# speedinghzl/DSRG

Hardware: AMD Instinct MI355X
Metric: images/sec DSRG train step (VGG16 321x321, 21-class) (higher is better)
Workload: dtype bf16 backbone (fp32 master weights) + f32/f64 supervision path

## Files before the change

### dsrg_amd/csrc/conv_igemm.hip

```cpp
#include "common.h"
#include <algorithm>
#include <cstdlib>
#include <cstring>
#include <functional>
#include <map>
#include <mutex>
#include <queue>
#include <vector>

namespace dsrg {
namespace {
typedef __attribute__((ext_vector_type(8))) __bf16 bf16x8;
typedef __attribute__((ext_vector_type(2))) __bf16 bf16x2;
typedef __attribute__((ext_vector_type(2))) float f32x2;
typedef __attribute__((ext_vector_type(16))) float f32x16;
typedef __attribute__((address_space(3))) void lds_void;

constexpr int kBM = 256, kBN = 256;
constexpr int kOutRow = 128 * 2 + 16;
constexpr int kOutWave = 64 * kOutRow;
constexpr uint32_t kOob = 0x80000000u;
constexpr int kRowTab = 8 * kOutWave;
constexpr int kRowTabBytes = kBM * 4;

__device__ __forceinline__ void wait_vm_lgkm_barrier() {
    asm volatile("s_waitcnt vmcnt(0) lgkmcnt(0)\n\ts_barrier" ::: "memory");
}

template <int BK, int NST> struct ICfg {
    static constexpr int ROW = BK * 2;
    static constexpr int CPR = ROW / 16;
    static constexpr int RPI = 1024 / ROW;
    static constexpr int IPW = 256 / RPI / 8;
    static constexpr int STAGE = (kBM + kBN) * ROW;
    static constexpr int KS = BK / 16;
    static constexpr int SPC = 64 / BK;
    static constexpr int AHEAD = NST - 1;
    static_assert(NST * STAGE <= kRowTab, "the row table sits behind the stages");
    static constexpr size_t LDS = (size_t)kRowTab + kRowTabBytes;
    __device__ static constexpr int swz(int r) { return BK == 64 ? (r >> 1) & 7 : (r >> 2) & 3; }
};

// ... 36 lines not shown
}
__device__ __forceinline__ uint32_t dropout_bytes(uint32_t e4, uint32_t seed_lo, uint32_t seed_hi) {
    return fmix32(fmix32(e4 ^ seed_lo) + seed_hi);
}

__device__ __forceinline__ uint32_t pack2(float lo, float hi) {
    f32x2 v = {lo, hi};
    bf16x2 b = __builtin_convertvector(v, bf16x2);
    return *reinterpret_cast<uint32_t *>(&b);
}

template <int N> __device__ __forceinline__ void wait_vm_barrier() {
    asm volatile("s_waitcnt vmcnt(%0)\n\ts_barrier" ::"n"(N) : "memory");
}

template <int BK, int NST, bool EARLY = false>
__device__ __forceinline__ void conv_igemm_body(const IgemmArgs &a, const int bid, const int nblk) {
    using C = ICfg<BK, NST>;
    extern __shared__ __attribute__((aligned(16))) unsigned char ig_lds[];
    const int tid = threadIdx.x, lane = tid & 63;
    const int wv = __builtin_amdgcn_readfirstlane(tid >> 6);
    const int l31 = lane & 31, kgrp = lane >> 5;
    const int wn = wv >> 2, wm = wv & 3;

    int grp, tm, tn;
    if (a.xcd_mix) {
        const int id = bid, xcd = id & 7, k = id >> 3;
        const int cm = (a.tiles_m - xcd + 7) >> 3, per_group = cm * a.tiles_n;
        if (cm <= 0 || k >= per_group * a.ngroups) return;
        grp = k / per_group;
        const int r = k - grp * per_group, tml = r / a.tiles_n;
        tn = r - tml * a.tiles_n;
        tm = xcd + 8 * tml;
    } else {
        const int total = nblk, id = bid;
        const int q = total >> 3, r = total & 7, xcd = id & 7, k = id >> 3;
        int t = (xcd < r ? xcd * (q + 1) : r * (q + 1) + (xcd - r) * q) + k;
// ... 100 lines not shown
        if (taps == 9) { dy = tap / 3 - 1; dx = tap - (tap / 3) * 3 - 1; }
        const int xc = a.cpp ? (int)((0x610u >> (2 * (cc / a.cpp))) & 3u) * a.cpp + cc % a.cpp : cc;
        const int toff = (dy * G.dil * W + dx * G.dil) * xrow + xc * 128 + h * C::ROW;
        unsigned char *P = ig_lds + stage * C::STAGE + wv * (32 * C::ROW);
        unsigned char *Wt = P + kBM * C::ROW;
#pragma unroll
        for (int i = 0; i < C::IPW; i++) {
            const uint32_t vo = ((pvalid[i] >> tap) & 1u) ? pbase[i] + (uint32_t)toff : kOob;
            __builtin_amdgcn_raw_ptr_buffer_load_lds(rx, (lds_void *)(P + i * (C::RPI * C::ROW)), 16, vo, 0, 0, 0);
        }
#pragma unroll
        for (int i = 0; i < C::IPW; i++)
            __builtin_amdgcn_raw_ptr_buffer_load_lds(rw, (lds_void *)(Wt + i * (C::RPI * C::ROW)), 16, wbase[i], s_real * C::ROW, 0, 0);
    };

    f32x16 acc[4][2];
#pragma unroll
    for (int i = 0; i < 4; i++)
#pragma unroll
        for (int j = 0; j < 2; j++)
#pragma unroll
            for (int r = 0; r < 16; r++) acc[i][j][r] = 0.0f;

    const int sw = C::swz(l31);
    const uint32_t rowoff = (uint32_t)l31 * C::ROW;
    uint32_t choff[C::KS];
#pragma unroll
    for (int ks = 0; ks < C::KS; ks++) choff[ks] = rowoff + (uint32_t)(((ks * 2 + kgrp) ^ sw) << 4);

    const bool active = n0 + wn * 128 < a.Cout;
    constexpr int LPS = 2 * C::IPW;
    if (EARLY) {
        static_assert(!EARLY || NST == 2, "the early-barrier schedule is written for two stages");
        bf16x8 af[2][4], bfr[2][2];
        const bool late = a.stagger && wv >= 4 && active;
        issue(0, 0);
        if (nsteps > 1) { issue(1, 1); wait_vm_barrier<LPS>(); } else { wait_vm_barrier<0>(); }
        if (active) {
            const unsigned char *P = ig_lds + wm * (64 * C::ROW), *Wt = ig_lds + kBM * C::ROW + wn * (128 * C::ROW);
#pragma unroll
            for (int i = 0; i < 4; i++) af[0][i] = *reinterpret_cast<const bf16x8 *>(Wt + i * (32 * C::ROW) + choff[0]);
#pragma unroll
            for (int j = 0; j < 2; j++) bfr[0][j] = *reinterpret_cast<const bf16x8 *>(P + j * (32 * C::ROW) + choff[0]);
        }
        for (int s = 0; s < nsteps; s++) {
            const int stage = s & 1;
            const bool next = s + 1 < nsteps, more = s + 2 < nsteps;
            if (!active) {
                if (next) { wait_vm_lgkm_barrier(); if (more) issue(stage, s + 2); }
                continue;
            }
            const unsigned char *P = ig_lds + stage * C::STAGE + wm * (64 * C::ROW);
            const unsigned char *Wt = ig_lds + stage * C::STAGE + kBM * C::ROW + wn * (128 * C::ROW);
            const unsigned char *Pn = ig_lds + (stage ^ 1) * C::STAGE + wm * (64 * C::ROW);
            const unsigned char *Wn = ig_lds + (stage ^ 1) * C::STAGE + kBM * C::ROW + wn * (128 * C::ROW);
#pragma unroll
            for (int ks = 0; ks < C::KS; ks++) {
                if (ks + 1 < C::KS) {
#pragma unroll
                    for (int i = 0; i < 4; i++) af[(ks + 1) & 1][i] = *reinterpret_cast<const bf16x8 *>(Wt + i * (32 * C::ROW) + choff[ks + 1 < C::KS ? ks + 1 : 0]);
#pragma unroll
                    for (int j = 0; j < 2; j++) bfr[(ks + 1) & 1][j] = *reinterpret_cast<const bf16x8 *>(P + j * (32 * C::ROW) + choff[ks + 1 < C::KS ? ks + 1 : 0]);
                } else if (next) {
                    wait_vm_lgkm_barrier();
                    if (more && !late) issue(stage, s + 2);
#pragma unroll
                    for (int i = 0; i < 4; i++) af[C::KS & 1][i] = *reinterpret_cast<const bf16x8 *>(Wn + i * (32 * C::ROW) + choff[0]);
#pragma unroll
                    for (int j = 0; j < 2; j++) bfr[C::KS & 1][j] = *reinterpret_cast<const bf16x8 *>(Pn + j * (32 * C::ROW) + choff[0]);
                }
                __builtin_amdgcn_sched_barrier(0);
#pragma unroll
                for (int i = 0; i < 4; i++)
#pragma unroll
                    for (int j = 0; j < 2; j++)
                        acc[i][j] = __builtin_amdgcn_mfma_f32_32x32x16_bf16(af[ks & 1][i], bfr[ks & 1][j], acc[i][j], 0, 0, 0);
                __builtin_amdgcn_sched_barrier(0);
                if (ks == C::KS - 1 && more && late) issue(stage, s + 2);
            }
        }
    } else {
#pragma unroll
    for (int p = 0; p < C::AHEAD; p++)
        if (p < nsteps) issue(p, p);
    int stage = 0;
    for (int s = 0; s < nsteps; s++) {
        if (C::AHEAD >= 3 && s + 2 < nsteps) wait_vm_barrier<2 * LPS>();
        else if (C::AHEAD >= 2 && s + 1 < nsteps) wait_vm_barrier<LPS>();
        else wait_vm_barrier<0>();
        const bool more = s + C::AHEAD < nsteps, late = a.stagger && wv >= 4 && active;
        const int nstage = stage == 0 ? NST - 1 : stage - 1;
        if (more && !late) issue(nstage, s + C::AHEAD);
        if (active) {
        const unsigned char *P = ig_lds + stage * C::STAGE + wm * (64 * C::ROW);
        const unsigned char *Wt = ig_lds + stage * C::STAGE + kBM * C::ROW + wn * (128 * C::ROW);
        bf16x8 af[2][4], bfr[2][2];
#pragma unroll
        for (int i = 0; i < 4; i++) af[0][i] = *reinterpret_cast<const bf16x8 *>(Wt + i * (32 * C::ROW) + choff[0]);
#pragma unroll
        for (int j = 0; j < 2; j++) bfr[0][j] = *reinterpret_cast<const bf16x8 *>(P + j * (32 * C::ROW) + choff[0]);
#pragma unroll
        for (int ks = 0; ks < C::KS; ks++) {
            if (ks + 1 < C::KS) {
#pragma unroll
                for (int i = 0; i < 4; i++) af[(ks + 1) & 1][i] = *reinterpret_cast<const bf16x8 *>(Wt + i * (32 * C::ROW) + choff[(ks + 1) % C::KS]);
#pragma unroll
                for (int j = 0; j < 2; j++) bfr[(ks + 1) & 1][j] = *reinterpret_cast<const bf16x8 *>(P + j * (32 * C::ROW) + choff[(ks + 1) % C::KS]);
            }
            __builtin_amdgcn_sched_barrier(0);
#pragma unroll
            for (int i = 0; i < 4; i++)
#pragma unroll
                for (int j = 0; j < 2; j++)
                    acc[i][j] = __builtin_amdgcn_mfma_f32_32x32x16_bf16(af[ks & 1][i], bfr[ks & 1][j], acc[i][j], 0, 0, 0);
            __builtin_amdgcn_sched_barrier(0);
            if (ks == 0 && more && late) issue(nstage, s + C::AHEAD);
        }
        }
        stage = stage + 1 == NST ? 0 : stage + 1;
    }
    }
    __syncthreads();
    if (!active) return;

    unsigned char *O = ig_lds + wv * kOutWave;
    const int nw = n0 + wn * 128;
    if (a.out_f32) {
        float *y32 = reinterpret_cast<float *>(G.y);
        const float floor32 = a.relu ? 0.0f : -__builtin_inff();
#pragma unroll
        for (int j = 0; j < 2; j++) {
            const int m = row_pixel(wm * 64 + j * 32 + l31);
#pragma unroll
            for (int i = 0; i < 4; i++)
#pragma unroll
                for (int q = 0; q < 4; q++) {
                    const int n = nw + i * 32 + q * 8 + kgrp * 4;
                    float4 b4 = make_float4(0.f, 0.f, 0.f, 0.f);
                    if (G.bias) b4 = *reinterpret_cast<const float4 *>(G.bias + n);
                    const float4 v = make_float4(fmaxf(acc[i][j][q * 4 + 0] + b4.x, floor32), fmaxf(acc[i][j][q * 4 + 1] + b4.y, floor32),
                                                 fmaxf(acc[i][j][q * 4 + 2] + b4.z, floor32), fmaxf(acc[i][j][q * 4 + 3] + b4.w, floor32));
                    if (m >= 0) *reinterpret_cast<float4 *>(y32 + (size_t)m * a.Cout + n) = v;
                }
        }
        return;
    }
    const rsrc_t rb = make_rsrc(G.bias, G.bias ? (size_t)a.Cout * 4 : 0);
    const float floor_ = (a.relu && !G.res) ? 0.0f : -__builtin_inff();
    const uint32_t seed_g = a.seed_lo + (uint32_t)grp * 0x9E3779B9u;
    float bias_r[4][4][4];
#pragma unroll
    for (int i = 0; i < 4; i++)
#pragma unroll
        for (int q = 0; q < 4; q++)
#pragma unroll
            for (int e = 0; e < 4; e++)
                bias_r[i][q][e] = ld_f32(rb, (uint32_t)(nw + i * 32 + q * 8 + kgrp * 4 + e) * 4u);
#pragma unroll
    for (int i = 0; i < 4; i++) {
#pragma unroll
        for (int q = 0; q < 4; q++) {
            const int nl = i * 32 + q * 8 + kgrp * 4;
            const float4 b4 = make_float4(bias_r[i][q][0], bias_r[i][q][1], bias_r[i][q][2], bias_r[i][q][3]);
#pragma unroll
            for (int j = 0; j < 2; j++) {
                float v0 = acc[i][j][q * 4 + 0] + b4.x, v1 = acc[i][j][q * 4 + 1] + b4.y;
                float v2 = acc[i][j][q * 4 + 2] + b4.z, v3 = acc[i][j][q * 4 + 3] + b4.w;
                v0 = fmaxf(v0, floor_) * a.out_scale; v1 = fmaxf(v1, floor_) * a.out_scale;
                v2 = fmaxf(v2, floor_) * a.out_scale; v3 = fmaxf(v3, floor_) * a.out_scale;
                if (a.drop_thresh) {
                    const uint32_t m = cls ? (uint32_t)rowpix[wm * 64 + j * 32 + l31] : (uint32_t)(m0 + wm * 64 + j * 32 + l31);
                    const uint32_t h = dropout_bytes((m * (uint32_t)a.Cout + (uint32_t)(nw + nl)) >> 2, seed_g, a.seed_hi);
                    v0 = (h & 0xffu) >= a.drop_thresh ? v0 * a.drop_scale : 0.0f;
                    v1 = ((h >> 8) & 0xffu) >= a.drop_thresh ? v1 * a.drop_scale : 0.0f;
                    v2 = ((h >> 16) & 0xffu) >= a.drop_thresh ? v2 * a.drop_scale : 0.0f;
                    v3 = (h >> 24) >= a.drop_thresh ? v3 * a.drop_scale : 0.0f;
                }
                *reinterpret_cast<uint2 *>(O + (j * 32 + l31) * kOutRow + nl * 2) = make_uint2(pack2(v0, v1), pack2(v2, v3));
            }
        }
    }
    const bool chv = nw + (lane & 15) * 8 < a.Cout;
    if (G.res) {
        const float floor2 = a.relu ? 0.0f : -__builtin_inff();
#pragma unroll
        for (int h = 0; h < 2; h++) {
            uint4 rs[8], mk8[8];
#pragma unroll
            for (int it = 0; it < 8; it++) {
                const int m = row_pixel(wm * 64 + (h * 8 + it) * 4 + (lane >> 4));
                const size_t at = (size_t)m * a.Cout + nw + (lane & 15) * 8;
                rs[it] = (m >= 0 && chv) ? *reinterpret_cast<const uint4 *>(G.res + at) : make_uint4(0, 0, 0, 0);
                mk8[it] = !G.mask ? make_uint4(0x3f803f80u, 0x3f803f80u, 0x3f803f80u, 0x3f803f80u)
                                  : ((m >= 0 && chv) ? *reinterpret_cast<const uint4 *>(G.mask + at) : make_uint4(0, 0, 0, 0));
// ... 71 lines not shown
        }
        __syncthreads();
        if (wm == 0) {
            const float *s0 = reinterpret_cast<const float *>(ig_lds + (wn * 4 + 0) * kOutWave);
            const float *s1 = reinterpret_cast<const float *>(ig_lds + (wn * 4 + 1) * kOutWave);
            const float *s2 = reinterpret_cast<const float *>(ig_lds + (wn * 4 + 2) * kOutWave);
            const float *s3 = reinterpret_cast<const float *>(ig_lds + (wn * 4 + 3) * kOutWave);
            float *dst = G.colsum + (size_t)tm * a.Cout + nw;
            dst[lane] = (s0[lane] + s1[lane]) + (s2[lane] + s3[lane]);
            if (nw + lane + 64 < a.Cout) dst[lane + 64] = (s0[lane + 64] + s1[lane + 64]) + (s2[lane + 64] + s3[lane + 64]);
        }
    }
}


__global__ __launch_bounds__(512, 2) void conv_igemm_kernel_64x2(IgemmArgs a) { conv_igemm_body<64, 2>(a, (int)blockIdx.x, (int)gridDim.x); }
__global__ __launch_bounds__(512, 2) void conv_igemm_kernel_64x2e(IgemmArgs a) { conv_igemm_body<64, 2, true>(a, (int)blockIdx.x, (int)gridDim.x); }
__global__ __launch_bounds__(512, 2) void conv_igemm_kernel_32x4(IgemmArgs a) { conv_igemm_body<32, 4>(a, (int)blockIdx.x, (int)gridDim.x); }

struct IgemmSkArgs {
    IgemmArgs base;
    float *ws;
    uint32_t *flags;
    int units, tiles_total;
};
constexpr int kSkParts = 4;
using f32x4v = decltype(__builtin_amdgcn_raw_buffer_load_b128(rsrc_t(), 0, 0, 0));

__global__ __launch_bounds__(512, 2) void conv_igemm_sk_kernel(IgemmSkArgs k) {
    using C = ICfg<64, 2>;
    const IgemmArgs &a = k.base;
    extern __shared__ __attribute__((aligned(16))) unsigned char ig_lds[];
    const int tid = threadIdx.x, lane = tid & 63;
    const int wv = __builtin_amdgcn_readfirstlane(tid >> 6);
    const int l31 = lane & 31, kgrp = lane >> 5;
    const int wn = wv >> 2, wm = wv & 3;
    int unit;
    {
        const int total = (int)gridDim.x, id = (int)blockIdx.x;
        const int q = total >> 3, r = total & 7, xcd = id & 7, kk = id >> 3;
        unit = (xcd < r ? xcd * (q + 1) : r * (q + 1) + (xcd - r) * q) + kk;
    }
    const int taps = a.taps, Cin = a.Cin, W = a.W, H = a.H;
    const int ktot = taps * Cin;
    const int nsteps = (Cin >> 6) * taps;
    const long long total_steps = (long long)k.tiles_total * nsteps;
    auto unit_start = [&](int u) { return (long long)u * total_steps / k.units; };
    const long long g1 = unit_start(unit + 1);
    const int sw = C::swz(l31);
    const uint32_t rowoff = (uint32_t)l31 * C::ROW;
    uint32_t choff[C::KS];
#pragma unroll
    for (int ks = 0; ks < C::KS; ks++) choff[ks] = rowoff + (uint32_t)(((ks * 2 + kgrp) ^ sw) << 4);
    const rsrc_t rws = make_rsrc(k.ws, (size_t)k.units * 32 * 512 * 16);
    const float floor_ = a.relu ? 0.0f : -__builtin_inff();

    for (long long g = unit_start(unit); g < g1;) {
        const int tile = (int)(g / nsteps);
        const int sb = (int)(g - (long long)tile * nsteps);
        const int se = (int)min((long long)nsteps, sb + (g1 - g));
        int t = tile;
        const int grp = t / a.tiles_per_group;
        t -= grp * a.tiles_per_group;
        const int tm = t / a.tiles_n, tn = t - tm * a.tiles_n;
        const int m0 = tm * kBM, n0 = tn * kBN;
        const IgemmGroup G = a.g[grp];
        const rsrc_t rx = make_rsrc(G.x, (size_t)a.M * Cin * 2);
        const rsrc_t rw = make_rsrc(G.w, (size_t)a.Cout * ktot * 2);
// ... 32 lines not shown
            const int toff = (dy * G.dil * W + dx * G.dil) * Cin * 2 + cc * 128;
            unsigned char *P = ig_lds + stage * C::STAGE + wv * (32 * C::ROW);
            unsigned char *Wt = P + kBM * C::ROW;
#pragma unroll
            for (int i = 0; i < C::IPW; i++) {
                const uint32_t bits = (i < 2 ? pvalid01 : pvalid23) >> (16 * (i & 1) + tap);
                const uint32_t off = ((pbase0 + (uint32_t)(i * C::RPI * Cin * 2)) ^ ((i & 1) ? 64u : 0u)) + (uint32_t)toff;
                __builtin_amdgcn_raw_ptr_buffer_load_lds(rx, (lds_void *)(P + i * (C::RPI * C::ROW)), 16, (bits & 1u) ? off : kOob, 0, 0, 0);
            }
#pragma unroll
            for (int i = 0; i < C::IPW; i++)
                __builtin_amdgcn_raw_ptr_buffer_load_lds(rw, (lds_void *)(Wt + i * (C::RPI * C::ROW)), 16, (i & 1) ? wbase0 ^ 64u : wbase0,
                                                         (uint32_t)s * C::ROW + (uint32_t)(i * C::RPI * ktot * 2), 0, 0);
        };

        f32x16 acc[4][2];
#pragma unroll
        for (int i = 0; i < 4; i++)
#pragma unroll
            for (int j = 0; j < 2; j++)
#pragma unroll
                for (int r = 0; r < 16; r++) acc[i][j][r] = 0.0f;

        issue(0, sb);
        for (int s = sb; s < se; s++) {
            const int stage = (s - sb) & 1;
            wait_vm_barrier<0>();
            const bool more = s + 1 < se, late = wv >= 4 && active;
            if (more && !late) issue(stage ^ 1, s + 1);
            if (active) {
                const unsigned char *P = ig_lds + stage * C::STAGE + wm * (64 * C::ROW);
                const unsigned char *Wt = ig_lds + stage * C::STAGE + kBM * C::ROW + wn * (128 * C::ROW);
                bf16x8 af[2][4], bfr[2][2];
#pragma unroll
                for (int i = 0; i < 4; i++) af[0][i] = *reinterpret_cast<const bf16x8 *>(Wt + i * (32 * C::ROW) + choff[0]);
#pragma unroll
                for (int j = 0; j < 2; j++) bfr[0][j] = *reinterpret_cast<const bf16x8 *>(P + j * (32 * C::ROW) + choff[0]);
#pragma unroll
                for (int ks = 0; ks < C::KS; ks++) {
                    if (ks + 1 < C::KS) {
#pragma unroll
                        for (int i = 0; i < 4; i++) af[(ks + 1) & 1][i] = *reinterpret_cast<const bf16x8 *>(Wt + i * (32 * C::ROW) + choff[(ks + 1) % C::KS]);
#pragma unroll
                        for (int j = 0; j < 2; j++) bfr[(ks + 1) & 1][j] = *reinterpret_cast<const bf16x8 *>(P + j * (32 * C::ROW) + choff[(ks + 1) % C::KS]);
                    }
                    __builtin_amdgcn_sched_barrier(0);
#pragma unroll
                    for (int i = 0; i < 4; i++)
#pragma unroll
                        for (int j = 0; j < 2; j++)
                            acc[i][j] = __builtin_amdgcn_mfma_f32_32x32x16_bf16(af[ks & 1][i], bfr[ks & 1][j], acc[i][j], 0, 0, 0);
                    __builtin_amdgcn_sched_barrier(0);
                    if (ks == 0 && more && late) issue(stage ^ 1, s + 1);
                }
            }
        }
        __syncthreads();

        if (sb != 0) {
            if (active) {
#pragma unroll
                for (int i = 0; i < 4; i++)
#pragma unroll
                    for (int j = 0; j < 2; j++)
#pragma unroll
                        for (int q = 0; q < 4; q++) {
                            f32x4v v = {__float_as_uint(acc[i][j][q * 4 + 0]), __float_as_uint(acc[i][j][q * 4 + 1]),
                                        __float_as_uint(acc[i][j][q * 4 + 2]), __float_as_uint(acc[i][j][q * 4 + 3])};
                            __builtin_amdgcn_raw_buffer_store_b128(v, rws, (uint32_t)(((i * 2 + j) * 4 + q) * 512 + tid) * 16u,
                                                                   (uint32_t)unit * (32u * 512u * 16u), 16);
                        }
            }
            asm volatile("s_waitcnt vmcnt(0)" ::: "memory");
            __syncthreads();
            if (tid == 0) __hip_atomic_store(k.flags + unit, 1u, __ATOMIC_RELAXED, __HIP_MEMORY_SCOPE_AGENT);
        } else {
            bool ok = true;
            int nparts = 0;
            if (se != nsteps) {
                const long long tile_end = (long long)(tile + 1) * nsteps;
                while (unit + 1 + nparts < k.units && unit_start(unit + 1 + nparts) < tile_end) nparts++;
                volatile int &sk_ok = *reinterpret_cast<volatile int *>(ig_lds);
                if (tid == 0) {
                    int good = nparts <= kSkParts ? 1 : 0;
                    for (int p = 0; p < nparts && good; p++) {
                        unsigned spins = 0;
// ... 7 lines not shown
                    sk_ok = good;
                }
                __syncthreads();
                ok = sk_ok != 0;
                __syncthreads();
            }
            if (active) {
                const float poison = ok ? 0.0f : __builtin_nanf("");
                unsigned char *O = ig_lds + wv * kOutWave;
                const int nw = n0 + wn * 128;
                const rsrc_t rb = make_rsrc(G.bias, G.bias ? (size_t)a.Cout * 4 : 0);
                const uint32_t seed_g = a.seed_lo + (uint32_t)grp * 0x9E3779B9u;
                f32x4v shares[2][kSkParts];
                float bq[2][4];
                auto fetch = [&](int gi, f32x4v (&dst)[kSkParts], float (&bias4)[4]) {
                    const int i = gi >> 3, q = (gi >> 1) & 3, j = gi & 1;
                    const uint32_t off = (uint32_t)(((i * 2 + j) * 4 + q) * 512 + tid) * 16u;
#pragma unroll
                    for (int p = 0; p < kSkParts; p++)
                        dst[p] = __builtin_amdgcn_raw_buffer_load_b128(rws, p < nparts ? off : kOob, (uint32_t)(unit + 1 + p) * (32u * 512u * 16u), 0);
#pragma unroll
                    for (int e = 0; e < 4; e++) bias4[e] = ld_f32(rb, (uint32_t)(nw + i * 32 + q * 8 + kgrp * 4 + e) * 4u);
                };
                fetch(0, shares[0], bq[0]);
#pragma unroll
                for (int gi = 0; gi < 32; gi++) {
                    const int i = gi >> 3, q = (gi >> 1) & 3, j = gi & 1;
                    if (gi + 1 < 32) fetch(gi + 1, shares[(gi + 1) & 1], bq[(gi + 1) & 1]);
                    __builtin_amdgcn_sched_barrier(0);
                    const int nl = i * 32 + q * 8 + kgrp * 4;
                    float s0 = acc[i][j][q * 4 + 0], s1 = acc[i][j][q * 4 + 1], s2 = acc[i][j][q * 4 + 2], s3 = acc[i][j][q * 4 + 3];
#pragma unroll
                    for (int p = 0; p < kSkParts; p++) {
                        const f32x4v pv = shares[gi & 1][p];
                        s0 += __uint_as_float(pv[0]); s1 += __uint_as_float(pv[1]); s2 += __uint_as_float(pv[2]); s3 += __uint_as_float(pv[3]);
                    }
                    float v0 = s0 + bq[gi & 1][0], v1 = s1 + bq[gi & 1][1], v2 = s2 + bq[gi & 1][2], v3 = s3 + bq[gi & 1][3];
                    v0 = fmaxf(v0, floor_) + poison; v1 = fmaxf(v1, floor_) + poison; v2 = fmaxf(v2, floor_) + poison; v3 = fmaxf(v3, floor_) + poison;
                    if (a.drop_thresh) {
                        const uint32_t m = (uint32_t)(m0 + wm * 64 + j * 32 + l31);
                        const uint32_t h = dropout_bytes((m * (uint32_t)a.Cout + (uint32_t)(nw + nl)) >> 2, seed_g, a.seed_hi);
                        v0 = (h & 0xffu) >= a.drop_thresh ? v0 * a.drop_scale : 0.0f;
                        v1 = ((h >> 8) & 0xffu) >= a.drop_thresh ? v1 * a.drop_scale : 0.0f;
                        v2 = ((h >> 16) & 0xffu) >= a.drop_thresh ? v2 * a.drop_scale : 0.0f;
                        v3 = (h >> 24) >= a.drop_thresh ? v3 * a.drop_scale : 0.0f;
                    }
                    *reinterpret_cast<uint2 *>(O + (j * 32 + l31) * kOutRow + nl * 2) = make_uint2(pack2(v0, v1), pack2(v2, v3));
                    __builtin_amdgcn_sched_barrier(0);
                }
#pragma unroll 4
                for (int it = 0; it < 16; it++) {
                    const int p = it * 4 + (lane >> 4), ch = lane & 15;
                    const int m = m0 + wm * 64 + p;
                    const uint4 v = *reinterpret_cast<const uint4 *>(O + p * kOutRow + ch * 16);
                    if (m < a.M) *reinterpret_cast<uint4 *>(G.y + (size_t)m * a.Cout + nw + ch * 8) = v;
                }
            }
        }
        g += se - sb;
        __syncthreads();
    }
}
// ... 217 lines not shown

__global__ __launch_bounds__(512, 2) void conv_igemm_wgrad_kernel(IgemmWgradArgs a) { conv_igemm_wgrad_body(a, (int)blockIdx.x, (int)gridDim.x); }

struct IgemmBwdArgs {
    IgemmArgs d;
    IgemmWgradArgs w;
    int nd, nd_pad, nw;
    int w_first, nw_pad;
};
__global__ __launch_bounds__(512, 2) void conv_igemm_bwd_kernel(IgemmBwdArgs a) {
    const int id = (int)blockIdx.x;
    if (a.w_first) {
        if (id < a.nw_pad) {
            if (id < a.nw) conv_igemm_wgrad_body(a.w, id, a.nw);
        } else if (id - a.nw_pad < a.nd) {
            conv_igemm_body<64, 2>(a.d, id - a.nw_pad, a.nd);
        }
        return;
    }
    if (id < a.nd_pad) {
        if (id < a.nd) conv_igemm_body<64, 2>(a.d, id, a.nd);
    } else {
        conv_igemm_wgrad_body(a.w, id - a.nd_pad, a.nw);
    }
}

struct WgradReduceArgs {
    const float *part[4];
    void *gw[4];
    int ksplit;
    size_t n4;
    const float *scale;
    size_t per_o4;
};
template <bool BF16_OUT>
__global__ __launch_bounds__(256) void conv_igemm_wgrad_reduce_kernel(WgradReduceArgs a) {
// ... 54 lines not shown
    }
}

}

bool conv_igemm_supported(int cin, int cout, int k) {
    return (k == 1 || k == 3) && cin >= 64 && cin % 64 == 0 && cout >= 128 && cout % 128 == 0;
}
static bool conv_igemm_launchable(int cin, int cout, int k) {
    return (k == 1 || k == 3) && cin >= 64 && cin % 64 == 0 && (cout == 64 || (cout >= 128 && cout % 128 == 0));
}

std::atomic<int> g_igemm_variant{-1};
static int igemm_variant() {
    const int v = g_igemm_variant.load(std::memory_order_relaxed);
    return v < 0 ? 3 : v;
}

static int igemm_cus() {
    static const int n = [] {
        int dev = 0, c = 0;
        if (hipGetDevice(&dev) != hipSuccess || hipDeviceGetAttribute(&c, hipDeviceAttributeMultiprocessorCount, dev) != hipSuccess || c < 8) c = 256;
        return c;
    }();
    return n;
}
size_t conv_igemm_workspace() { return (size_t)igemm_cus() * (32 * 512 * 16) + ((size_t)igemm_cus() + 1 + 63) / 64 * 256; }

struct ColsumArgs {
    const float *part[4];
    float *out[4];
// ... 144 lines not shown
        a.out_f32 = 1;
    }
    a.skip_taps = igemm_variant() != 6;
    const bool fused_bwd = mask || colsum || t_res;
    if (t_res && (colsum || ngroups != 1 || drop_p != 0.0f || t_split_cin))
        return set_error(DSRG_ERR_UNSUPPORTED, "conv_igemm: a residual goes with one group, no column sums, no dropout");
    a.ngroups = ngroups; a.B = B; a.H = H; a.W = W; a.Cin = cin; a.Cout = cout; a.taps = k * k; a.relu = relu; a.M = (int)M;
    a.tiles_m = (int)((M + kBM - 1) / kBM);
    a.tiles_n = (cout + kBN - 1) / kBN;
    a.tiles_per_group = a.tiles_m * a.tiles_n;
    if (drop_p < 0.0f || drop_p >= 1.0f) return set_error(DSRG_ERR_INVALID, "conv_igemm: 0 <= dropout probability < 1");
    a.drop_thresh = (uint32_t)(drop_p * 256.0f + 0.5f);
    if (a.drop_thresh > 255) a.drop_thresh = 255;
    a.drop_scale = 256.0f / (float)(256 - (int)a.drop_thresh);
    a.seed_lo = (uint32_t)seed; a.seed_hi = (uint32_t)(seed >> 32);
    static LdsGrant grant[3];
    const int variant = igemm_variant() == 2 ? 1 : 0;
    a.stagger = igemm_variant() >= 3;
    const bool default_form = igemm_variant() == 3 || igemm_variant() == 8 || igemm_variant() == 9;
    const dim3 block(512);
    const int units = igemm_cus(), tiles_total = a.tiles_per_group * ngroups, nsteps = (cin / 64) * k * k;
    const bool sk_wins = tiles_total * 100 <= units * 60, sk_forced = igemm_variant() == 4;
    if (!fused_bwd && t_split_cin == 0 && cout % 128 == 0 && workspace && workspace_bytes >= conv_igemm_workspace() && ((default_form && sk_wins) || sk_forced) &&
        (long long)tiles_total * nsteps >= (long long)units * 8 && tiles_total * 3 >= units) {
        IgemmSkArgs sk;
        sk.base = a;
        sk.base.stagger = 1;
        sk.ws = static_cast<float *>(workspace);
        sk.flags = reinterpret_cast<uint32_t *>(static_cast<unsigned char *>(workspace) + (size_t)units * (32 * 512 * 16));
        sk.units = units;
        sk.tiles_total = tiles_total;
        constexpr size_t lds = ICfg<64, 2>::LDS;
        if (int rc = ensure_dynamic_lds(reinterpret_cast<const void *>(&conv_igemm_sk_kernel), lds, grant[2])) return rc;
        DSRG_HIP_CHECK(hipMemsetAsync(sk.flags, 0, sizeof(uint32_t) * ((size_t)units + 1), stream));
        hipLaunchKernelGGL(conv_igemm_sk_kernel, dim3(units), block, lds, stream, sk);
        DSRG_LAUNCH_CHECK();
        return DSRG_OK;
    }
    for (int g = 0; g < ngroups; g++)
        if (a.skip_taps && k == 3 && a.g[g].dil >= 3) a.xcd_mix = 1;
    const bool rows_ok = a.xcd_mix && W <= kBM && conv_igemm_row_tiles(H, W);
    if (a.xcd_mix && igemm_variant() != 8 && H <= 255 && W <= 255) {
        struct Key { int B, H, W, d[4], n, rows; bool operator<(const Key &o) const { return memcmp(this, &o, sizeof(Key)) < 0; } };
        static std::map<Key, bool> memo;
        static std::mutex memo_mutex;
        Key key;
        memset(&key, 0, sizeof(key));
        key.B = B; key.H = H; key.W = W; key.n = ngroups; key.rows = rows_ok;
// ... 25 lines not shown
        }
    }
    if (!a.cls_tiles && rows_ok) {
        a.row_tiles = 1;
        a.rows_per_tile = kBM / W;
        a.bands = (H + a.rows_per_tile - 1) / a.rows_per_tile;
        a.tiles_m = B * a.bands;
        a.tiles_per_group = a.tiles_m * a.tiles_n;
    }
    const dim3 grid(a.xcd_mix ? 8 * ngroups * ((a.tiles_m + 7) / 8) * a.tiles_n : a.tiles_per_group * ngroups);
    if (t_prep_d) {
        *t_prep_d = a;
        *t_prep_grid = (int)grid.x;
        return DSRG_OK;
    }
    if (igemm_variant() == 5) {
        static LdsGrant grant_e;
        constexpr size_t lds = ICfg<64, 2>::LDS;
        if (int rc = ensure_dynamic_lds(reinterpret_cast<const void *>(&conv_igemm_kernel_64x2e), lds, grant_e)) return rc;
        hipLaunchKernelGGL(conv_igemm_kernel_64x2e, grid, block, lds, stream, a);
    } else if (variant == 0) {
        constexpr size_t lds = ICfg<64, 2>::LDS;
        if (int rc = ensure_dynamic_lds(reinterpret_cast<const void *>(&conv_igemm_kernel_64x2), lds, grant[0])) return rc;
        hipLaunchKernelGGL(conv_igemm_kernel_64x2, grid, block, lds, stream, a);
    } else {
        constexpr size_t lds = ICfg<32, 4>::LDS;
        if (int rc = ensure_dynamic_lds(reinterpret_cast<const void *>(&conv_igemm_kernel_32x4), lds, grant[1])) return rc;
        hipLaunchKernelGGL(conv_igemm_kernel_32x4, grid, block, lds, stream, a);
    }
    DSRG_LAUNCH_CHECK();
    if (colsum) {
        const float *parts[4];
        for (int g = 0; g < ngroups; g++) parts[g] = a.g[g].colsum;
        if (int rc = launch_igemm_colsum(parts, colsum, ngroups, a.tiles_m, cout, stream)) return rc;
    }
    return DSRG_OK;
}


int launch_conv_igemm_split(const void *x3, const void *w, const float *bias, float *y, int dil, int B, int H, int W, int cin, int cout, int k,
                            int relu, hipStream_t stream) {
    if (!conv_igemm_supported(cin, cout, k) || (long long)B * H * W * 3 * cin * 2 >= 0x7fffffffLL)
        return set_error(DSRG_ERR_UNSUPPORTED, "conv_igemm_split: shape not supported");
    const void *xp[1] = {x3}, *wp[1] = {w};
// ... 263 lines not shown
```

Baseline: 1966.

## Switch implicit-GEMM conv inner loop to 16x16x32 MFMA with register ring prefetch

Replaces the 32x32x16 bf16 MFMA tiling (4x2 f32x16 accumulators) with 16x16x32 MFMA over an 8x4 grid of f32x4 accumulators. Weight fragments stream from LDS through a small register ring read several steps ahead. The data and split-K kernels share a new helper for this, which changes fragment offsets, epilogue indexing and the workspace layout. The 32x4 and early-barrier variants are removed, leaving a single two-stage schedule. The aim is denser MFMA issue and better overlap of LDS reads with math, at the cost of more LDS read instructions and different register pressure.

```diff
diff --git a/dsrg_amd/csrc/conv_igemm.hip b/dsrg_amd/csrc/conv_igemm.hip
--- a/dsrg_amd/csrc/conv_igemm.hip
+++ b/dsrg_amd/csrc/conv_igemm.hip
@@ -14,6 +14,7 @@
 typedef __attribute__((ext_vector_type(2))) __bf16 bf16x2;
 typedef __attribute__((ext_vector_type(2))) float f32x2;
 typedef __attribute__((ext_vector_type(16))) float f32x16;
+typedef __attribute__((ext_vector_type(4))) float f32x4;
 typedef __attribute__((address_space(3))) void lds_void;
 
 constexpr int kBM = 256, kBN = 256;
@@ -22,10 +23,6 @@
 constexpr uint32_t kOob = 0x80000000u;
 constexpr int kRowTab = 8 * kOutWave;
 constexpr int kRowTabBytes = kBM * 4;
-
-__device__ __forceinline__ void wait_vm_lgkm_barrier() {
-    asm volatile("s_waitcnt vmcnt(0) lgkmcnt(0)\n\ts_barrier" ::: "memory");
-}
 
 template <int BK, int NST> struct ICfg {
     static constexpr int ROW = BK * 2;
@@ -92,13 +89,46 @@
     asm volatile("s_waitcnt vmcnt(%0)\n\ts_barrier" ::"n"(N) : "memory");
 }
 
-template <int BK, int NST, bool EARLY = false>
+constexpr int kAhead = 3;
+struct IgemmFrag {
+    uint32_t choff[2];
+    __device__ __forceinline__ explicit IgemmFrag(int lane) {
+        using C = ICfg<64, 2>;
+        const int l15 = lane & 15, g4 = lane >> 4;
+#pragma unroll
+        for (int sl = 0; sl < 2; sl++) choff[sl] = (uint32_t)l15 * C::ROW + (uint32_t)(((sl * 4 + g4) ^ C::swz(l15)) << 4);
+    }
+};
+template <class LateIssue>
+__device__ __forceinline__ void igemm_mma_step(const unsigned char *P, const unsigned char *Wt, const IgemmFrag &fr, f32x4 (&acc)[8][4],
+                                               const bool late, LateIssue &&late_issue) {
+    using C = ICfg<64, 2>;
+    constexpr int RING = kAhead + 1;
+    bf16x8 bq[2][4], ar[RING];
+    auto read_w = [&](int u) { return *reinterpret_cast<const bf16x8 *>(Wt + (u & 7) * (16 * C::ROW) + fr.choff[u >> 3]); };
+#pragma unroll
+    for (int j = 0; j < 4; j++) bq[0][j] = *reinterpret_cast<const bf16x8 *>(P + j * (16 * C::ROW) + fr.choff[0]);
+#pragma unroll
+    for (int u = 0; u < kAhead; u++) ar[u] = read_w(u);
+#pragma unroll
+    for (int u = 0; u < 16; u++) {
+        if (u + kAhead < 16) ar[(u + kAhead) % RING] = read_w(u + kAhead);
+        if (u < 4) bq[1][u] = *reinterpret_cast<const bf16x8 *>(P + u * (16 * C::ROW) + fr.choff[1]);
+        __builtin_amdgcn_sched_barrier(0);
+#pragma unroll
+        for (int j = 0; j < 4; j++)
+            acc[u & 7][j] = __builtin_amdgcn_mfma_f32_16x16x32_bf16(ar[u % RING], bq[u >> 3][j], acc[u & 7][j], 0, 0, 0);
+        __builtin_amdgcn_sched_barrier(0);
+        if (u == 3 && late) late_issue();
+    }
+}
+
 __device__ __forceinline__ void conv_igemm_body(const IgemmArgs &a, const int bid, const int nblk) {
-    using C = ICfg<BK, NST>;
+    using C = ICfg<64, 2>;
     extern __shared__ __attribute__((aligned(16))) unsigned char ig_lds[];
     const int tid = threadIdx.x, lane = tid & 63;
     const int wv = __builtin_amdgcn_readfirstlane(tid >> 6);
-    const int l31 = lane & 31, kgrp = lane >> 5;
+    const int l15 = lane & 15, g4 = lane >> 4;
     const int wn = wv >> 2, wm = wv & 3;
 
     int grp, tm, tn;
@@ -229,111 +259,32 @@
             __builtin_amdgcn_raw_ptr_buffer_load_lds(rw, (lds_void *)(Wt + i * (C::RPI * C::ROW)), 16, wbase[i], s_real * C::ROW, 0, 0);
     };
 
-    f32x16 acc[4][2];
-#pragma unroll
-    for (int i = 0; i < 4; i++)
-#pragma unroll
-        for (int j = 0; j < 2; j++)
-#pragma unroll
-            for (int r = 0; r < 16; r++) acc[i][j][r] = 0.0f;
-
-    const int sw = C::swz(l31);
-    const uint32_t rowoff = (uint32_t)l31 * C::ROW;
-    uint32_t choff[C::KS];
-#pragma unroll
-    for (int ks = 0; ks < C::KS; ks++) choff[ks] = rowoff + (uint32_t)(((ks * 2 + kgrp) ^ sw) << 4);
-
+    f32x4 acc[8][4];
+#pragma unroll
+    for (int i = 0; i < 8; i++)
+#pragma unroll
+        for (int j = 0; j < 4; j++)
+#pragma unroll
+            for (int r = 0; r < 4; r++) acc[i][j][r] = 0.0f;
+
+    const IgemmFrag fr(lane);
     const bool active = n0 + wn * 128 < a.Cout;
-    constexpr int LPS = 2 * C::IPW;
-    if (EARLY) {
-        static_assert(!EARLY || NST == 2, "the early-barrier schedule is written for two stages");
-        bf16x8 af[2][4], bfr[2][2];
-        const bool late = a.stagger && wv >= 4 && active;
-        issue(0, 0);
-        if (nsteps > 1) { issue(1, 1); wait_vm_barrier<LPS>(); } else { wait_vm_barrier<0>(); }
-        if (active) {
-            const unsigned char *P = ig_lds + wm * (64 * C::ROW), *Wt = ig_lds + kBM * C::ROW + wn * (128 * C::ROW);
-#pragma unroll
-            for (int i = 0; i < 4; i++) af[0][i] = *reinterpret_cast<const bf16x8 *>(Wt + i * (32 * C::ROW) + choff[0]);
-#pragma unroll
-            for (int j = 0; j < 2; j++) bfr[0][j] = *reinterpret_cast<const bf16x8 *>(P + j * (32 * C::ROW) + choff[0]);
-        }
+    const bool late = a.stagger && wv >= 4 && active;
+    if (nsteps > 0) issue(0, 0);
+    if (!active) {
+        for (int s = 0; s < nsteps; s++) {
+            wait_vm_barrier<0>();
+            if (s + 1 < nsteps) issue((s & 1) ^ 1, s + 1);
+        }
+    } else {
         for (int s = 0; s < nsteps; s++) {
             const int stage = s & 1;
-            const bool next = s + 1 < nsteps, more = s + 2 < nsteps;
-            if (!active) {
-                if (next) { wait_vm_lgkm_barrier(); if (more) issue(stage, s + 2); }
-                continue;
-            }
-            const unsigned char *P = ig_lds + stage * C::STAGE + wm * (64 * C::ROW);
-            const unsigned char *Wt = ig_lds + stage * C::STAGE + kBM * C::ROW + wn * (128 * C::ROW);
-            const unsigned char *Pn = ig_lds + (stage ^ 1) * C::STAGE + wm * (64 * C::ROW);
-            const unsigned char *Wn = ig_lds + (stage ^ 1) * C::STAGE + kBM * C::ROW + wn * (128 * C::ROW);
-#pragma unroll
-            for (int ks = 0; ks < C::KS; ks++) {
-                if (ks + 1 < C::KS) {
-#pragma unroll
-                    for (int i = 0; i < 4; i++) af[(ks + 1) & 1][i] = *reinterpret_cast<const bf16x8 *>(Wt + i * (32 * C::ROW) + choff[ks + 1 < C::KS ? ks + 1 : 0]);
-#pragma unroll
-                    for (int j = 0; j < 2; j++) bfr[(ks + 1) & 1][j] = *reinterpret_cast<const bf16x8 *>(P + j * (32 * C::ROW) + choff[ks + 1 < C::KS ? ks + 1 : 0]);
-                } else if (next) {
-                    wait_vm_lgkm_barrier();
-                    if (more && !late) issue(stage, s + 2);
-#pragma unroll
-                    for (int i = 0; i < 4; i++) af[C::KS & 1][i] = *reinterpret_cast<const bf16x8 *>(Wn + i * (32 * C::ROW) + choff[0]);
-#pragma unroll
-                    for (int j = 0; j < 2; j++) bfr[C::KS & 1][j] = *reinterpret_cast<const bf16x8 *>(Pn + j * (32 * C::ROW) + choff[0]);
-                }
-                __builtin_amdgcn_sched_barrier(0);
-#pragma unroll
-                for (int i = 0; i < 4; i++)
-#pragma unroll
-                    for (int j = 0; j < 2; j++)
-                        acc[i][j] = __builtin_amdgcn_mfma_f32_32x32x16_bf16(af[ks & 1][i], bfr[ks & 1][j], acc[i][j], 0, 0, 0);
-                __builtin_amdgcn_sched_barrier(0);
-                if (ks == C::KS - 1 && more && late) issue(stage, s + 2);
-            }
-        }
-    } else {
-#pragma unroll
-    for (int p = 0; p < C::AHEAD; p++)
-        if (p < nsteps) issue(p, p);
-    int stage = 0;
-    for (int s = 0; s < nsteps; s++) {
-        if (C::AHEAD >= 3 && s + 2 < nsteps) wait_vm_barrier<2 * LPS>();
-        else if (C::AHEAD >= 2 && s + 1 < nsteps) wait_vm_barrier<LPS>();
-        else wait_vm_barrier<0>();
-        const bool more = s + C::AHEAD < nsteps, late = a.stagger && wv >= 4 && active;
-        const int nstage = stage == 0 ? NST - 1 : stage - 1;
-        if (more && !late) issue(nstage, s + C::AHEAD);
-        if (active) {
-        const unsigned char *P = ig_lds + stage * C::STAGE + wm * (64 * C::ROW);
-        const unsigned char *Wt = ig_lds + stage * C::STAGE + kBM * C::ROW + wn * (128 * C::ROW);
-        bf16x8 af[2][4], bfr[2][2];
-#pragma unroll
-        for (int i = 0; i < 4; i++) af[0][i] = *reinterpret_cast<const bf16x8 *>(Wt + i * (32 * C::ROW) + choff[0]);
-#pragma unroll
-        for (int j = 0; j < 2; j++) bfr[0][j] = *reinterpret_cast<const bf16x8 *>(P + j * (32 * C::ROW) + choff[0]);
-#pragma unroll
-        for (int ks = 0; ks < C::KS; ks++) {
-            if (ks + 1 < C::KS) {
-#pragma unroll
-                for (int i = 0; i < 4; i++) af[(ks + 1) & 1][i] = *reinterpret_cast<const bf16x8 *>(Wt + i * (32 * C::ROW) + choff[(ks + 1) % C::KS]);
-#pragma unroll
-                for (int j = 0; j < 2; j++) bfr[(ks + 1) & 1][j] = *reinterpret_cast<const bf16x8 *>(P + j * (32 * C::ROW) + choff[(ks + 1) % C::KS]);
-            }
-            __builtin_amdgcn_sched_barrier(0);
-#pragma unroll
-            for (int i = 0; i < 4; i++)
-#pragma unroll
-                for (int j = 0; j < 2; j++)
-                    acc[i][j] = __builtin_amdgcn_mfma_f32_32x32x16_bf16(af[ks & 1][i], bfr[ks & 1][j], acc[i][j], 0, 0, 0);
-            __builtin_amdgcn_sched_barrier(0);
-            if (ks == 0 && more && late) issue(nstage, s + C::AHEAD);
-        }
-        }
-        stage = stage + 1 == NST ? 0 : stage + 1;
-    }
+            wait_vm_barrier<0>();
+            const bool more = s + 1 < nsteps;
+            if (more && !late) issue(stage ^ 1, s + 1);
+            igemm_mma_step(ig_lds + stage * C::STAGE + wm * (64 * C::ROW), ig_lds + stage * C::STAGE + kBM * C::ROW + wn * (128 * C::ROW), fr, acc,
+                           more && late, [&]() { issue(stage ^ 1, s + 1); });
+        }
     }
     __syncthreads();
     if (!active) return;
@@ -344,55 +295,46 @@
         float *y32 = reinterpret_cast<float *>(G.y);
         const float floor32 = a.relu ? 0.0f : -__builtin_inff();
 #pragma unroll
-        for (int j = 0; j < 2; j++) {
-            const int m = row_pixel(wm * 64 + j * 32 + l31);
-#pragma unroll
-            for (int i = 0; i < 4; i++)
-#pragma unroll
-                for (int q = 0; q < 4; q++) {
-                    const int n = nw + i * 32 + q * 8 + kgrp * 4;
-                    float4 b4 = make_float4(0.f, 0.f, 0.f, 0.f);
-                    if (G.bias) b4 = *reinterpret_cast<const float4 *>(G.bias + n);
-                    const float4 v = make_float4(fmaxf(acc[i][j][q * 4 + 0] + b4.x, floor32), fmaxf(acc[i][j][q * 4 + 1] + b4.y, floor32),
-                                                 fmaxf(acc[i][j][q * 4 + 2] + b4.z, floor32), fmaxf(acc[i][j][q * 4 + 3] + b4.w, floor32));
-                    if (m >= 0) *reinterpret_cast<float4 *>(y32 + (size_t)m * a.Cout + n) = v;
-                }
+        for (int j = 0; j < 4; j++) {
+            const int m = row_pixel(wm * 64 + j * 16 + l15);
+#pragma unroll
+            for (int i = 0; i < 8; i++) {
+                const int n = nw + i * 16 + g4 * 4;
+                float4 b4 = make_float4(0.f, 0.f, 0.f, 0.f);
+                if (G.bias) b4 = *reinterpret_cast<const float4 *>(G.bias + n);
+                const float4 v = make_float4(fmaxf(acc[i][j][0] + b4.x, floor32), fmaxf(acc[i][j][1] + b4.y, floor32),
+                                             fmaxf(acc[i][j][2] + b4.z, floor32), fmaxf(acc[i][j][3] + b4.w, floor32));
+                if (m >= 0) *reinterpret_cast<float4 *>(y32 + (size_t)m * a.Cout + n) = v;
+            }
         }
         return;
     }
     const rsrc_t rb = make_rsrc(G.bias, G.bias ? (size_t)a.Cout * 4 : 0);
     const float floor_ = (a.relu && !G.res) ? 0.0f : -__builtin_inff();
     const uint32_t seed_g = a.seed_lo + (uint32_t)grp * 0x9E3779B9u;
-    float bias_r[4][4][4];
-#pragma unroll
-    for (int i = 0; i < 4; i++)
-#pragma unroll
-        for (int q = 0; q < 4; q++)
-#pragma unroll
-            for (int e = 0; e < 4; e++)
-                bias_r[i][q][e] = ld_f32(rb, (uint32_t)(nw + i * 32 + q * 8 + kgrp * 4 + e) * 4u);
-#pragma unroll
-    for (int i = 0; i < 4; i++) {
-#pragma unroll
-        for (int q = 0; q < 4; q++) {
-            const int nl = i * 32 + q * 8 + kgrp * 4;
-            const float4 b4 = make_float4(bias_r[i][q][0], bias_r[i][q][1], bias_r[i][q][2], bias_r[i][q][3]);
-#pragma unroll
-            for (int j = 0; j < 2; j++) {
-                float v0 = acc[i][j][q * 4 + 0] + b4.x, v1 = acc[i][j][q * 4 + 1] + b4.y;
-                float v2 = acc[i][j][q * 4 + 2] + b4.z, v3 = acc[i][j][q * 4 + 3] + b4.w;
-                v0 = fmaxf(v0, floor_) * a.out_scale; v1 = fmaxf(v1, floor_) * a.out_scale;
-                v2 = fmaxf(v2, floor_) * a.out_scale; v3 = fmaxf(v3, floor_) * a.out_scale;
-                if (a.drop_thresh) {
-                    const uint32_t m = cls ? (uint32_t)rowpix[wm * 64 + j * 32 + l31] : (uint32_t)(m0 + wm * 64 + j * 32 + l31);
-                    const uint32_t h = dropout_bytes((m * (uint32_t)a.Cout + (uint32_t)(nw + nl)) >> 2, seed_g, a.seed_hi);
-                    v0 = (h & 0xffu) >= a.drop_thresh ? v0 * a.drop_scale : 0.0f;
-                    v1 = ((h >> 8) & 0xffu) >= a.drop_thresh ? v1 * a.drop_scale : 0.0f;
-                    v2 = ((h >> 16) & 0xffu) >= a.drop_thresh ? v2 * a.drop_scale : 0.0f;
-                    v3 = (h >> 24) >= a.drop_thresh ? v3 * a.drop_scale : 0.0f;
-                }
-                *reinterpret_cast<uint2 *>(O + (j * 32 + l31) * kOutRow + nl * 2) = make_uint2(pack2(v0, v1), pack2(v2, v3));
-            }
+    float bias_r[8][4];
+#pragma unroll
+    for (int i = 0; i < 8; i++)
+#pragma unroll
+        for (int e = 0; e < 4; e++) bias_r[i][e] = ld_f32(rb, (uint32_t)(nw + i * 16 + g4 * 4 + e) * 4u);
+#pragma unroll
+    for (int i = 0; i < 8; i++) {
+        const int nl = i * 16 + g4 * 4;
+#pragma unroll
+        for (int j = 0; j < 4; j++) {
+            float v0 = acc[i][j][0] + bias_r[i][0], v1 = acc[i][j][1] + bias_r[i][1];
+            float v2 = acc[i][j][2] + bias_r[i][2], v3 = acc[i][j][3] + bias_r[i][3];
+            v0 = fmaxf(v0, floor_) * a.out_scale; v1 = fmaxf(v1, floor_) * a.out_scale;
+            v2 = fmaxf(v2, floor_) * a.out_scale; v3 = fmaxf(v3, floor_) * a.out_scale;
+            if (a.drop_thresh) {
+                const uint32_t m = cls ? (uint32_t)rowpix[wm * 64 + j * 16 + l15] : (uint32_t)(m0 + wm * 64 + j * 16 + l15);
+                const uint32_t h = dropout_bytes((m * (uint32_t)a.Cout + (uint32_t)(nw + nl)) >> 2, seed_g, a.seed_hi);
+                v0 = (h & 0xffu) >= a.drop_thresh ? v0 * a.drop_scale : 0.0f;
+                v1 = ((h >> 8) & 0xffu) >= a.drop_thresh ? v1 * a.drop_scale : 0.0f;
+                v2 = ((h >> 16) & 0xffu) >= a.drop_thresh ? v2 * a.drop_scale : 0.0f;
+                v3 = (h >> 24) >= a.drop_thresh ? v3 * a.drop_scale : 0.0f;
+            }
+            *reinterpret_cast<uint2 *>(O + (j * 16 + l15) * kOutRow + nl * 2) = make_uint2(pack2(v0, v1), pack2(v2, v3));
         }
     }
     const bool chv = nw + (lane & 15) * 8 < a.Cout;
@@ -494,9 +436,7 @@
 }
 
 
-__global__ __launch_bounds__(512, 2) void conv_igemm_kernel_64x2(IgemmArgs a) { conv_igemm_body<64, 2>(a, (int)blockIdx.x, (int)gridDim.x); }
-__global__ __launch_bounds__(512, 2) void conv_igemm_kernel_64x2e(IgemmArgs a) { conv_igemm_body<64, 2, true>(a, (int)blockIdx.x, (int)gridDim.x); }
-__global__ __launch_bounds__(512, 2) void conv_igemm_kernel_32x4(IgemmArgs a) { conv_igemm_body<32, 4>(a, (int)blockIdx.x, (int)gridDim.x); }
+__global__ __launch_bounds__(512, 2) void conv_igemm_kernel_64x2(IgemmArgs a) { conv_igemm_body(a, (int)blockIdx.x, (int)gridDim.x); }
 
 struct IgemmSkArgs {
     IgemmArgs base;
@@ -513,7 +453,7 @@
     extern __shared__ __attribute__((aligned(16))) unsigned char ig_lds[];
     const int tid = threadIdx.x, lane = tid & 63;
     const int wv = __builtin_amdgcn_readfirstlane(tid >> 6);
-    const int l31 = lane & 31, kgrp = lane >> 5;
+    const int l15 = lane & 15, g4 = lane >> 4;
     const int wn = wv >> 2, wm = wv & 3;
     int unit;
     {
@@ -527,11 +467,7 @@
     const long long total_steps = (long long)k.tiles_total * nsteps;
     auto unit_start = [&](int u) { return (long long)u * total_steps / k.units; };
     const long long g1 = unit_start(unit + 1);
-    const int sw = C::swz(l31);
-    const uint32_t rowoff = (uint32_t)l31 * C::ROW;
-    uint32_t choff[C::KS];
-#pragma unroll
-    for (int ks = 0; ks < C::KS; ks++) choff[ks] = rowoff + (uint32_t)(((ks * 2 + kgrp) ^ sw) << 4);
+    const IgemmFrag fr(lane);
     const rsrc_t rws = make_rsrc(k.ws, (size_t)k.units * 32 * 512 * 16);
     const float floor_ = a.relu ? 0.0f : -__builtin_inff();
 
@@ -594,45 +530,28 @@
                                                          (uint32_t)s * C::ROW + (uint32_t)(i * C::RPI * ktot * 2), 0, 0);
         };
 
-        f32x16 acc[4][2];
-#pragma unroll
-        for (int i = 0; i < 4; i++)
-#pragma unroll
-            for (int j = 0; j < 2; j++)
-#pragma unroll
-                for (int r = 0; r < 16; r++) acc[i][j][r] = 0.0f;
+        f32x4 acc[8][4];
+#pragma unroll
+        for (int i = 0; i < 8; i++)
+#pragma unroll
+            for (int j = 0; j < 4; j++)
+#pragma unroll
+                for (int r = 0; r < 4; r++) acc[i][j][r] = 0.0f;
 
         issue(0, sb);
-        for (int s = sb; s < se; s++) {
-            const int stage = (s - sb) & 1;
-            wait_vm_barrier<0>();
-            const bool more = s + 1 < se, late = wv >= 4 && active;
-            if (more && !late) issue(stage ^ 1, s + 1);
-            if (active) {
-                const unsigned char *P = ig_lds + stage * C::STAGE + wm * (64 * C::ROW);
-                const unsigned char *Wt = ig_lds + stage * C::STAGE + kBM * C::ROW + wn * (128 * C::ROW);
-                bf16x8 af[2][4], bfr[2][2];
-#pragma unroll
-                for (int i = 0; i < 4; i++) af[0][i] = *reinterpret_cast<const bf16x8 *>(Wt + i * (32 * C::ROW) + choff[0]);
-#pragma unroll
-                for (int j = 0; j < 2; j++) bfr[0][j] = *reinterpret_cast<const bf16x8 *>(P + j * (32 * C::ROW) + choff[0]);
-#pragma unroll
-                for (int ks = 0; ks < C::KS; ks++) {
-                    if (ks + 1 < C::KS) {
-#pragma unroll
-                        for (int i = 0; i < 4; i++) af[(ks + 1) & 1][i] = *reinterpret_cast<const bf16x8 *>(Wt + i * (32 * C::ROW) + choff[(ks + 1) % C::KS]);
-#pragma unroll
-                        for (int j = 0; j < 2; j++) bfr[(ks + 1) & 1][j] = *reinterpret_cast<const bf16x8 *>(P + j * (32 * C::ROW) + choff[(ks + 1) % C::KS]);
-                    }
-                    __builtin_amdgcn_sched_barrier(0);
-#pragma unroll
-                    for (int i = 0; i < 4; i++)
-#pragma unroll
-                        for (int j = 0; j < 2; j++)
-                            acc[i][j] = __builtin_amdgcn_mfma_f32_32x32x16_bf16(af[ks & 1][i], bfr[ks & 1][j], acc[i][j], 0, 0, 0);
-                    __builtin_amdgcn_sched_barrier(0);
-                    if (ks == 0 && more && late) issue(stage ^ 1, s + 1);
-                }
+        if (!active) {
+            for (int s = sb; s < se; s++) {
+                wait_vm_barrier<0>();
+                if (s + 1 < se) issue(((s - sb) & 1) ^ 1, s + 1);
+            }
+        } else {
+            for (int s = sb; s < se; s++) {
+                const int stage = (s - sb) & 1;
+                wait_vm_barrier<0>();
+                const bool more = s + 1 < se, late = wv >= 4;
+                if (more && !late) issue(stage ^ 1, s + 1);
+                igemm_mma_step(ig_lds + stage * C::STAGE + wm * (64 * C::ROW), ig_lds + stage * C::STAGE + kBM * C::ROW + wn * (128 * C::ROW), fr, acc,
+                               more && late, [&]() { issue(stage ^ 1, s + 1); });
             }
         }
         __syncthreads();
@@ -640,16 +559,13 @@
         if (sb != 0) {
             if (active) {
 #pragma unroll
-                for (int i = 0; i < 4; i++)
-#pragma unroll
-                    for (int j = 0; j < 2; j++)
-#pragma unroll
-                        for (int q = 0; q < 4; q++) {
-                            f32x4v v = {__float_as_uint(acc[i][j][q * 4 + 0]), __float_as_uint(acc[i][j][q * 4 + 1]),
-                                        __float_as_uint(acc[i][j][q * 4 + 2]), __float_as_uint(acc[i][j][q * 4 + 3])};
-                            __builtin_amdgcn_raw_buffer_store_b128(v, rws, (uint32_t)(((i * 2 + j) * 4 + q) * 512 + tid) * 16u,
-                                                                   (uint32_t)unit * (32u * 512u * 16u), 16);
-                        }
+                for (int i = 0; i < 8; i++)
+#pragma unroll
+                    for (int j = 0; j < 4; j++) {
+                        f32x4v v = {__float_as_uint(acc[i][j][0]), __float_as_uint(acc[i][j][1]), __float_as_uint(acc[i][j][2]), __float_as_uint(acc[i][j][3])};
+                        __builtin_amdgcn_raw_buffer_store_b128(v, rws, (uint32_t)((i * 4 + j) * 512 + tid) * 16u,
+                                                               (uint32_t)unit * (32u * 512u * 16u), 16);
+                    }
             }
             asm volatile("s_waitcnt vmcnt(0)" ::: "memory");
             __syncthreads();
@@ -687,22 +603,22 @@
                 f32x4v shares[2][kSkParts];
                 float bq[2][4];
                 auto fetch = [&](int gi, f32x4v (&dst)[kSkParts], float (&bias4)[4]) {
-                    const int i = gi >> 3, q = (gi >> 1) & 3, j = gi & 1;
-                    const uint32_t off = (uint32_t)(((i * 2 + j) * 4 + q) * 512 + tid) * 16u;
+                    const int i = gi >> 2;
+                    const uint32_t off = (uint32_t)(gi * 512 + tid) * 16u;
 #pragma unroll
                     for (int p = 0; p < kSkParts; p++)
                         dst[p] = __builtin_amdgcn_raw_buffer_load_b128(rws, p < nparts ? off : kOob, (uint32_t)(unit + 1 + p) * (32u * 512u * 16u), 0);
 #pragma unroll
-                    for (int e = 0; e < 4; e++) bias4[e] = ld_f32(rb, (uint32_t)(nw + i * 32 + q * 8 + kgrp * 4 + e) * 4u);
+                    for (int e = 0; e < 4; e++) bias4[e] = ld_f32(rb, (uint32_t)(nw + i * 16 + g4 * 4 + e) * 4u);
                 };
                 fetch(0, shares[0], bq[0]);
 #pragma unroll
                 for (int gi = 0; gi < 32; gi++) {
-                    const int i = gi >> 3, q = (gi >> 1) & 3, j = gi & 1;
+                    const int i = gi >> 2, j = gi & 3;
                     if (gi + 1 < 32) fetch(gi + 1, shares[(gi + 1) & 1], bq[(gi + 1) & 1]);
                     __builtin_amdgcn_sched_barrier(0);
-                    const int nl = i * 32 + q * 8 + kgrp * 4;
-                    float s0 = acc[i][j][q * 4 + 0], s1 = acc[i][j][q * 4 + 1], s2 = acc[i][j][q * 4 + 2], s3 = acc[i][j][q * 4 + 3];
+                    const int nl = i * 16 + g4 * 4;
+                    float s0 = acc[i][j][0], s1 = acc[i][j][1], s2 = acc[i][j][2], s3 = acc[i][j][3];
 #pragma unroll
                     for (int p = 0; p < kSkParts; p++) {
                         const f32x4v pv = shares[gi & 1][p];
@@ -711,14 +627,14 @@
                     float v0 = s0 + bq[gi & 1][0], v1 = s1 + bq[gi & 1][1], v2 = s2 + bq[gi & 1][2], v3 = s3 + bq[gi & 1][3];
                     v0 = fmaxf(v0, floor_) + poison; v1 = fmaxf(v1, floor_) + poison; v2 = fmaxf(v2, floor_) + poison; v3 = fmaxf(v3, floor_) + poison;
                     if (a.drop_thresh) {
-                        const uint32_t m = (uint32_t)(m0 + wm * 64 + j * 32 + l31);
+                        const uint32_t m = (uint32_t)(m0 + wm * 64 + j * 16 + l15);
                         const uint32_t h = dropout_bytes((m * (uint32_t)a.Cout + (uint32_t)(nw + nl)) >> 2, seed_g, a.seed_hi);
                         v0 = (h & 0xffu) >= a.drop_thresh ? v0 * a.drop_scale : 0.0f;
                         v1 = ((h >> 8) & 0xffu) >= a.drop_thresh ? v1 * a.drop_scale : 0.0f;
                         v2 = ((h >> 16) & 0xffu) >= a.drop_thresh ? v2 * a.drop_scale : 0.0f;
                         v3 = (h >> 24) >= a.drop_thresh ? v3 * a.drop_scale : 0.0f;
                     }
-                    *reinterpret_cast<uint2 *>(O + (j * 32 + l31) * kOutRow + nl * 2) = make_uint2(pack2(v0, v1), pack2(v2, v3));
+                    *reinterpret_cast<uint2 *>(O + (j * 16 + l15) * kOutRow + nl * 2) = make_uint2(pack2(v0, v1), pack2(v2, v3));
                     __builtin_amdgcn_sched_barrier(0);
                 }
 #pragma unroll 4
@@ -966,12 +882,12 @@
         if (id < a.nw_pad) {
             if (id < a.nw) conv_igemm_wgrad_body(a.w, id, a.nw);
         } else if (id - a.nw_pad < a.nd) {
-            conv_igemm_body<64, 2>(a.d, id - a.nw_pad, a.nd);
+            conv_igemm_body(a.d, id - a.nw_pad, a.nd);
         }
         return;
     }
     if (id < a.nd_pad) {
-        if (id < a.nd) conv_igemm_body<64, 2>(a.d, id, a.nd);
+        if (id < a.nd) conv_igemm_body(a.d, id, a.nd);
     } else {
         conv_igemm_wgrad_body(a.w, id - a.nd_pad, a.nw);
     }
@@ -1056,7 +972,7 @@
 std::atomic<int> g_igemm_variant{-1};
 static int igemm_variant() {
     const int v = g_igemm_variant.load(std::memory_order_relaxed);
-    return v < 0 ? 3 : v;
+    return (v < 0 || v == 2 || v == 5) ? 3 : v;
 }
 
 static int igemm_cus() {
@@ -1231,8 +1147,7 @@
     if (a.drop_thresh > 255) a.drop_thresh = 255;
     a.drop_scale = 256.0f / (float)(256 - (int)a.drop_thresh);
     a.seed_lo = (uint32_t)seed; a.seed_hi = (uint32_t)(seed >> 32);
-    static LdsGrant grant[3];
-    const int variant = igemm_variant() == 2 ? 1 : 0;
+    static LdsGrant grant[2];
     a.stagger = igemm_variant() >= 3;
     const bool default_form = igemm_variant() == 3 || igemm_variant() == 8 || igemm_variant() == 9;
     const dim3 block(512);
@@ -1248,7 +1163,7 @@
         sk.units = units;
         sk.tiles_total = tiles_total;
         constexpr size_t lds = ICfg<64, 2>::LDS;
-        if (int rc = ensure_dynamic_lds(reinterpret_cast<const void *>(&conv_igemm_sk_kernel), lds, grant[2])) return rc;
+        if (int rc = ensure_dynamic_lds(reinterpret_cast<const void *>(&conv_igemm_sk_kernel), lds, grant[1])) return rc;
         DSRG_HIP_CHECK(hipMemsetAsync(sk.flags, 0, sizeof(uint32_t) * ((size_t)units + 1), stream));
         hipLaunchKernelGGL(conv_igemm_sk_kernel, dim3(units), block, lds, stream, sk);
         DSRG_LAUNCH_CHECK();
@@ -1304,20 +1219,9 @@
         *t_prep_grid = (int)grid.x;
         return DSRG_OK;
     }
-    if (igemm_variant() == 5) {
-        static LdsGrant grant_e;
-        constexpr size_t lds = ICfg<64, 2>::LDS;
-        if (int rc = ensure_dynamic_lds(reinterpret_cast<const void *>(&conv_igemm_kernel_64x2e), lds, grant_e)) return rc;
-        hipLaunchKernelGGL(conv_igemm_kernel_64x2e, grid, block, lds, stream, a);
-    } else if (variant == 0) {
-        constexpr size_t lds = ICfg<64, 2>::LDS;
-        if (int rc = ensure_dynamic_lds(reinterpret_cast<const void *>(&conv_igemm_kernel_64x2), lds, grant[0])) return rc;
-        hipLaunchKernelGGL(conv_igemm_kernel_64x2, grid, block, lds, stream, a);
-    } else {
-        constexpr size_t lds = ICfg<32, 4>::LDS;
-        if (int rc = ensure_dynamic_lds(reinterpret_cast<const void *>(&conv_igemm_kernel_32x4), lds, grant[1])) return rc;
-        hipLaunchKernelGGL(conv_igemm_kernel_32x4, grid, block, lds, stream, a);
-    }
+    constexpr size_t lds = ICfg<64, 2>::LDS;
+    if (int rc = ensure_dynamic_lds(reinterpret_cast<const void *>(&conv_igemm_kernel_64x2), lds, grant[0])) return rc;
+    hipLaunchKernelGGL(conv_igemm_kernel_64x2, grid, block, lds, stream, a);
     DSRG_LAUNCH_CHECK();
     if (colsum) {
         const float *parts[4];
```

Measured after the change: 1987 (median of 6 runs). +1.1%, better.
